# lijrjyan/SDVAR

Measured on AMD Instinct MI355X. Metric: images/s (+ mean accepted tokens/step), VAR-d16 256^2 B=8, d12 draft + d16 verify, per GPU, higher is better.
Workload: dtype f32 (GEMM operands split into 2 fp16 planes to 2^-22, 3 fp16 MFMA products, fp32 accumulate); 1 GPU; BASELINE.json P1: VAR-d16 256^2 B=8/GPU, d12 draft + d16 verify, gamma=2, cfg=1.5 top_k=900 top_p=0.96, acceptance=natural, incl. VQVAE decode (overlapped with the next batch on a 2nd stream); verifier one round behind the draft once gamma = 1; parallelism=1 independent batch shards

## Files before the change

sdvar_amd/csrc/gemm.hip:

```cpp
#include "common.h"
#include "gemm_plan.h"

namespace sdvar {

enum { EPI_BIAS = 0, EPI_BIAS_GELU = 1, EPI_GATED_RES = 2, EPI_PARTIAL = 3 };

constexpr int BK = 32;
constexpr int LDS_STRIDE = BK + 4;

struct GemmArgs {
    const float* X; const float* W; const float* bias; float* out;
    const float* res; const float* gate;
    int M, N, K, ldx, ldo, ldres;
    int rows_per_gate, gate_stride;
    int split, k_per_split;
};

template <int BM, int BN, int WAVES_M, int WAVES_N, int EPI>
__global__ __launch_bounds__(256) void gemm_f32_nt_kernel(GemmArgs a) {
    static_assert(WAVES_M * WAVES_N == 4, "4 waves per workgroup");
    constexpr int WM = BM / WAVES_M, WN = BN / WAVES_N;
    constexpr int TM = WM / 32, TN = WN / 32;
    static_assert(TM >= 1 && TN >= 1, "wave tile too small");
    constexpr int XV = BM / 32, WV = BN / 32;
// ... 59 lines not shown
            for (int i = 0; i < TM; ++i) fa[i] = *reinterpret_cast<const f32x4*>(px + i * 32 * LDS_STRIDE + 8 * c);
#pragma unroll
            for (int j = 0; j < TN; ++j) fb[j] = *reinterpret_cast<const f32x4*>(pw + j * 32 * LDS_STRIDE + 8 * c);
#pragma unroll
            for (int e = 0; e < 4; ++e)
#pragma unroll
                for (int i = 0; i < TM; ++i)
#pragma unroll
                    for (int j = 0; j < TN; ++j)
                        acc[i][j] = __builtin_amdgcn_mfma_f32_32x32x2f32(fa[i][e], fb[j][e], acc[i][j], 0, 0, 0);
        }
        if (kt + 1 < nk) store_tile(buf ^ 1);
        __syncthreads();
    }

#pragma unroll
    for (int j = 0; j < TN; ++j) {
        const int n = n0 + wn * WN + j * 32 + li;
        if (n >= a.N) continue;
        const float bv = (EPI != EPI_PARTIAL && a.bias) ? a.bias[n] : 0.f;
        float* outp = (EPI == EPI_PARTIAL) ? a.out + (size_t)ks * a.M * a.ldo : a.out;
#pragma unroll
        for (int i = 0; i < TM; ++i) {
#pragma unroll
            for (int r = 0; r < 16; ++r) {
                const int m = m0 + wm * WM + i * 32 + (r & 3) + 8 * (r >> 2) + 4 * lh;
                if (m >= a.M) continue;
                float v = acc[i][j][r] + bv;
                if (EPI == EPI_BIAS_GELU) v = gelu_tanh(v);
                if (EPI == EPI_GATED_RES) {
                    const float g = a.gate[(size_t)(m / a.rows_per_gate) * a.gate_stride + n];
                    v = a.res[(size_t)m * a.ldres + n] + v * g;
                }
                outp[(size_t)m * a.ldo + n] = v;
            }
        }
    }
}

template <int EPI>
__global__ __launch_bounds__(256) void splitk_reduce_kernel(const float* __restrict__ ws, int split, const float* __restrict__ bias, float* out,
                                                            const float* res, const float* __restrict__ gate, int M, int N, int ldo, int ldres,
                                                            int rows_per_gate, int gate_stride) {
    const int nv = N >> 2;
    const size_t total = (size_t)M * nv, slab = (size_t)M * N;
    for (size_t i = (size_t)blockIdx.x * blockDim.x + threadIdx.x; i < total; i += (size_t)gridDim.x * blockDim.x) {
        const int m = (int)(i / nv), n = (int)(i % nv) * 4;
        f32x4 acc = *reinterpret_cast<const f32x4*>(ws + (size_t)m * N + n);
        for (int s = 1; s < split; ++s) {
            const f32x4 p = *reinterpret_cast<const f32x4*>(ws + s * slab + (size_t)m * N + n);
            acc[0] += p[0]; acc[1] += p[1]; acc[2] += p[2]; acc[3] += p[3];
        }
#pragma unroll
        for (int e = 0; e < 4; ++e) {
            float v = acc[e] + (bias ? bias[n + e] : 0.f);
            if (EPI == EPI_BIAS_GELU) v = gelu_tanh(v);
            if (EPI == EPI_GATED_RES) v = res[(size_t)m * ldres + n + e] + v * gate[(size_t)(m / rows_per_gate) * gate_stride + n + e];
            out[(size_t)m * ldo + n + e] = v;
        }
    }
}

static thread_local float* g_ws = nullptr;
constexpr size_t WS_FLOATS = (size_t)24 << 20;

static thread_local float* g_ws_model = nullptr;
float* set_splitk_workspace(float* p) { float* old = g_ws_model; g_ws_model = p; return old; }
size_t splitk_workspace_floats() { return WS_FLOATS; }

float* splitk_workspace(size_t* floats) {
    if (floats) *floats = WS_FLOATS;
    if (g_ws_model) return g_ws_model;
    if (!g_ws && hipMalloc((void**)&g_ws, WS_FLOATS * sizeof(float)) != hipSuccess) { set_error("split-K workspace allocation failed"); return nullptr; }
    return g_ws;
}

Variant g_variants[VAR_COUNT] = {
    {"gemm_h4_var", "SDVAR_GEMM_H4_VAR", 3, 0, 3, 3, false, false},
    {"gemm_h2_stages", "SDVAR_GEMM_H2_STAGES", 6, 2, 6, 6, false, false},
    {"gemm_small_pp", "SDVAR_GEMM_SMALL_PP", 2, 0, 2, 2, false, false},
    {"attn_pp_sched", "SDVAR_ATTN_PP_SCHED", 1, 0, 3, 1, false, false},
    {"conv_pp", "SDVAR_CONV_PP", 2, 0, 2, 2, true, false},
    {"conv_tap_reuse", "SDVAR_CONV_TAP_REUSE", 1, 0, 1, 1, true, false},
    {"rowblk", "SDVAR_ROWBLK", 1, 0, 2, 1, false, false},
    {"qkv_fuse", "SDVAR_NO_QKV_FUSE", 1, 0, 1, 1, false, true},
    {"gemm_v2", nullptr, 1, 0, 1, 1, false, false},
    {nullptr, nullptr, 0, 0, 768, 0, false, false},
    {nullptr, nullptr, 0, -64, 64, 0, false, false},
};

template <int BM, int BN, int WAVES_M, int WAVES_N, int EPI>
static int launch_f32_kernel(const GemmArgs& a, int grid, hipStream_t stream) {
    const size_t lds = 2 * (size_t)(BM + BN) * LDS_STRIDE * sizeof(float);
    static LdsOptIn opt_in;
    SDVAR_LDS_OPT_IN(opt_in, lds, (const void*)gemm_f32_nt_kernel<BM, BN, WAVES_M, WAVES_N, EPI>);
    hipLaunchKernelGGL((gemm_f32_nt_kernel<BM, BN, WAVES_M, WAVES_N, EPI>), dim3(grid), dim3(256), lds, stream, a);
    SDVAR_LAUNCH_CHECK();
    return SDVAR_OK;
}

static int launch_reduce(const GemmArgs& a, const float* ws, int split, int epi, hipStream_t stream) {
    return dispatch_epi(epi, [&](auto e) {
        hipLaunchKernelGGL(splitk_reduce_kernel<decltype(e)::value>, dim3(splitk_reduce_grid(a.M, a.N)), dim3(256), 0, stream, ws, split, a.bias, a.out, a.res, a.gate, a.M, a.N, a.ldo, a.ldres,
                           a.rows_per_gate, a.gate_stride);
        SDVAR_LAUNCH_CHECK();
        return SDVAR_OK;
    });
}

template <int BM, int BN, int WAVES_M, int WAVES_N>
static int launch_cfg(const GemmArgs& a, int epi, int split, hipStream_t stream) {
    const int tiles = ((a.M + BM - 1) / BM) * ((a.N + BN - 1) / BN);
    return launch_splitk(a, epi, split, tiles, nullptr,
                         [&](const GemmArgs& x, int grid, auto e) { return launch_f32_kernel<BM, BN, WAVES_M, WAVES_N, decltype(e)::value>(x, grid, stream); },
                         [&](const GemmArgs& x, const float* ws, int sp, int ep) { return launch_reduce(x, ws, sp, ep, stream); });
}

int gemm_f32_nt(const float* X, int ldx, const float* W, const float* bias, float* out, int ldo, int M, int N, int K, int epi,
                const float* res, int ldres, const float* gate, int rows_per_gate, int gate_stride, hipStream_t stream) {
    SDVAR_CHECK_ARG(X && W && out, "gemm: null operand");
    SDVAR_CHECK_ARG(M > 0 && N > 0 && K > 0 && K % BK == 0, "gemm: need K %% 32 == 0 (M=%d N=%d K=%d)", M, N, K);
    SDVAR_CHECK_ARG(ldx >= K && ldx % 4 == 0 && ldo >= N, "gemm: bad leading dims ldx=%d ldo=%d", ldx, ldo);
    SDVAR_CHECK_ARG(((uintptr_t)X % 16) == 0 && ((uintptr_t)W % 16) == 0, "gemm: operands must be 16-byte aligned");
    SDVAR_CHECK_ARG(epi >= EPI_BIAS && epi <= EPI_GATED_RES, "gemm: unknown epilogue %d", epi);
    if (epi == EPI_GATED_RES) SDVAR_CHECK_ARG(res && gate && rows_per_gate > 0 && ldres >= N, "gemm: gated-residual epilogue needs res/gate");
    const GemmArgs a{X, W, bias, out, res, gate, M, N, K, ldx, ldo, ldres, rows_per_gate > 0 ? rows_per_gate : 1, gate_stride, 1, K / BK};
    const GemmPlan p = plan_f32(M, N, K, WS_FLOATS);
    if (p.kernel == 32) return launch_cfg<32, 128, 1, 4>(a, epi, p.split, stream);
    if (p.kernel == 64) return launch_cfg<64, 128, 2, 2>(a, epi, p.split, stream);
    return launch_cfg<128, 128, 2, 2>(a, epi, p.split, stream);
}

}
```

sdvar_amd/csrc/gemm_f16x2.hip:

```cpp
#include <stdio.h>
#include <stdlib.h>

#include "common.h"
#include "gemm_plan.h"

namespace sdvar {

unsigned long long* debug_get_gemm_stamps();

typedef _Float16 f16x8 __attribute__((ext_vector_type(8)));
enum { HEPI_BIAS = 0, HEPI_BIAS_GELU_PLANES = 1, HEPI_GATED_RES = 2, HEPI_PARTIAL = 3, HEPI_QKV = 4 };

#ifdef SDVAR_TIMING_EXPERIMENTS
#define SDVAR_DBG(a, bit) ((a).dbg & (bit))
#else
#define SDVAR_DBG(a, bit) 0
#endif

constexpr int HBK = 32;
constexpr int HBN = 128;

struct QkvEpi {
    const float* scale_mul;
    float* q_out; uint16_t* k_cache; uint16_t* v_cache;
// ... 935 lines not shown
            else asm volatile("s_waitcnt vmcnt(0)" ::: "memory");
        }
        SDVAR_H4_SLOT(7);
        SDVAR_H4_MFMA(2, 0, if (p2) issue_w(t + 2, 2, 3), if (p2) issue_w(t + 2, 3, 4));
        SDVAR_H4_SLOT(8);
    }
    if (wm == 0) __builtin_amdgcn_s_barrier();
#ifdef SDVAR_V4_STAMPS
    wsr[2] = __builtin_amdgcn_s_memrealtime(); wsc[2] = __builtin_amdgcn_s_memtime();
    if (a.stamps && blockIdx.x == 0 && lane == 0 && (wave == 0 || wave == 4)) {
#pragma unroll
        for (int k = 0; k < 9; ++k) a.stamps[16 * (wave >> 2) + k] = stm[k];
    }
#endif
#undef SDVAR_H4_MFMA
#undef SDVAR_H4_SLOT
#undef SDVAR_H4_STAMP

    const float wsi = a.wsi ? *a.wsi : 1.0f;
    if (EPI == HEPI_QKV) {
        const int Cq = a.qk.H * 64, nw = n0 + wn * 64, which = nw / Cq, h = (nw - which * Cq) >> 6;
        if (nw >= a.N) return;
#pragma unroll
        for (int i = 0; i < 4; ++i) {
            const int m = m0 + wm * 128 + i * 32 + li;
            f32x16 v[2];
            float sq = qk_bias_sq(a, acc[i][0], v[0], wsi, nw + 4 * lh);
            sq += qk_bias_sq(a, acc[i][1], v[1], wsi, nw + 32 + 4 * lh);
            if (which != 2) sq += __shfl_xor(sq, 32, 64);
            qk_store_row<2>(a, v, sq, which, h, m, lh, 0);
        }
        return;
    }
    float* outp = (EPI == HEPI_PARTIAL) ? a.out + (size_t)ks * a.M * a.ldo : a.out;
    if (a.vec && n0 + BN <= a.N) {
#pragma unroll
        for (int j = 0; j < 2; ++j)
#pragma unroll
            for (int i = 0; i < 4; ++i) h_store_tile_fast<EPI>(a, outp, acc[i][j], wsi, m0 + wm * 128 + i * 32 + li, n0 + wn * 64 + j * 32 + 4 * lh);
    } else {
#pragma unroll
        for (int j = 0; j < 2; ++j)
#pragma unroll
            for (int i = 0; i < 4; ++i) h_store_tile<EPI>(a, outp, acc[i][j], wsi, m0 + wm * 128 + i * 32 + li, n0 + wn * 64 + j * 32 + 4 * lh);
    }
#ifdef SDVAR_V4_STAMPS
    if (a.stamps && lane == 0 && wave == 0 && (blockIdx.x == 0 || blockIdx.x == gridDim.x - 1)) {
        asm volatile("s_waitcnt vmcnt(0)" ::: "memory");
        wsr[3] = __builtin_amdgcn_s_memrealtime(); wsc[3] = __builtin_amdgcn_s_memtime();
        unsigned long long* o = a.stamps + 32 + (blockIdx.x == 0 ? 0 : 8);
#pragma unroll
        for (int k = 0; k < 4; ++k) { o[k] = wsr[k]; o[4 + k] = wsc[k]; }
    }
#endif
}

typedef float f32x4v __attribute__((ext_vector_type(4)));
#define SDVAR_MFMA3_16(acc, xh, xl, wh, wl)                                            \
    acc = __builtin_amdgcn_mfma_f32_16x16x32_f16(wh, xl, acc, 0, 0, 0);                \
    acc = __builtin_amdgcn_mfma_f32_16x16x32_f16(wl, xh, acc, 0, 0, 0);                \
    acc = __builtin_amdgcn_mfma_f32_16x16x32_f16(wh, xh, acc, 0, 0, 0)

template <int EPI>
__device__ __forceinline__ void h_store4(const GemmHArgs& a, float* outp, const f32x4v& acc, float wsi, int m, int n, bool fast) {
    if (m >= a.M || n >= a.N) return;
    if (!fast) {
#pragma unroll
        for (int e = 0; e < 4; ++e)
            if (n + e < a.N) h_store<EPI>(a, outp, acc[e], wsi, (EPI != HEPI_PARTIAL && a.bias) ? a.bias[n + e] : 0.f, m, n + e);
        return;
    }
    f32x4 v;
    if (EPI != HEPI_PARTIAL && a.bias) {
        const f32x4 bv = *reinterpret_cast<const f32x4*>(a.bias + n);
#pragma unroll
        for (int e = 0; e < 4; ++e) v[e] = __builtin_fmaf(acc[e], wsi, bv[e]);
    } else {
#pragma unroll
        for (int e = 0; e < 4; ++e) v[e] = acc[e] * wsi;
    }
    if (EPI == HEPI_BIAS_GELU_PLANES) {
        float gv[4];
#pragma unroll
        for (int e = 0; e < 4; ++e) gv[e] = gelu_tanh_h(v[e]);
        uint2 wh, wl;
        split4h_pk(gv, wh, wl);
        uint16_t* p0 = a.outp + kb_index(m, n, a.M);
        *reinterpret_cast<uint2*>(p0) = wh; *reinterpret_cast<uint2*>(p0 + a.ops) = wl;
        return;
    }
    if (EPI == HEPI_GATED_RES) {
        const f32x4 rv = *reinterpret_cast<const f32x4*>(a.res + (size_t)m * a.ldres + n);
        const f32x4 gt = *reinterpret_cast<const f32x4*>(a.gate + (size_t)(m / a.rows_per_gate) * a.gate_stride + n);
#pragma unroll
        for (int e = 0; e < 4; ++e) v[e] = rv[e] + v[e] * gt[e];
    }
    *reinterpret_cast<f32x4*>(outp + (size_t)m * a.ldo + n) = v;
}

template <int EPI>
__global__ __launch_bounds__(512, 2) void gemm_f16x2_v5_kernel(GemmHArgs a) {
    extern __shared__ __attribute__((aligned(16))) uint16_t hsm[];
    constexpr int BM = 256, BN = 256;
    const int tiles_m = (a.M + BM - 1) / BM, tiles_n = (a.N + BN - 1) / BN, ntile = tiles_m * tiles_n;
    const int ks = blockIdx.x / ntile;
    const int lid = xcd_remap(blockIdx.x - ks * ntile, ntile);
    const int G = 4, per_group = tiles_m * G;
    const int g = lid / per_group, rem = lid - g * per_group;
    const int gw = min(G, tiles_n - g * G);
    const int tm = rem / gw, tn = g * G + rem % gw;
    const int m0 = tm * BM, n0 = tn * BN;

    const int tid = threadIdx.x, lane = tid & 63, l15 = lane & 15, lq = lane >> 4;
    const int wave = __builtin_amdgcn_readfirstlane(tid >> 6);
    const int wm = wave >> 2, wn = wave & 3;
    const int kt0 = ks * a.k_per_split;
    const int nk = min(a.K / HBK - kt0, a.k_per_split);

    const int dpl = wave >> 2, drow0 = 64 * (wave & 3) + (lane >> 2);
    const int dch = (lane & 3) ^ ((lane >> 4) & 3);
    uint32_t vx[4], vw[4];
#pragma unroll
    for (int e = 0; e < 4; ++e) {
        vx[e] = (uint32_t)(min(m0 + drow0 + 16 * e, a.M - 1) * 32 + 8 * dch) * 2u;
        vw[e] = (uint32_t)(min(n0 + drow0 + 16 * e, a.N - 1) * 32 + 8 * dch) * 2u;
    }
    const char* const bx = reinterpret_cast<const char*>(a.X + (size_t)kt0 * a.M * 32 + (size_t)dpl * a.xps);
    const char* const bw = reinterpret_cast<const char*>(a.W + (size_t)kt0 * a.N * 32 + (size_t)dpl * a.wps);
    const uint32_t lds0 = SDVAR_LDS_ADDR(hsm);
    const uint32_t ldx = lds0 + (uint32_t)(dpl * 16384 + (64 * (wave & 3)) * 64), ldw = ldx + 32768u;
    auto issue_x = [&](int t) {
        const char* src = bx + (size_t)t * a.M * 64;
        const uint32_t dst = ldx + (uint32_t)(t & 1) * 65536u;
#pragma unroll
        for (int e = 0; e < 4; ++e) SDVAR_DMA16(vx[e], src, dst + 1024u * e);
    };
    auto issue_w = [&](int t) {
        const char* src = bw + (size_t)t * a.N * 64;
        const uint32_t dst = ldw + (uint32_t)(t & 1) * 65536u;
#pragma unroll
        for (int e = 0; e < 4; ++e) SDVAR_DMA16(vw[e], src, dst + 1024u * e);
    };

    f32x4v acc[8][4];
#pragma unroll
    for (int i = 0; i < 8; ++i)
#pragma unroll
        for (int j = 0; j < 4; ++j)
#pragma unroll
            for (int r = 0; r < 4; ++r) acc[i][j][r] = 0.f;

    const uint32_t fro = (uint32_t)(l15 * 64 + 16 * (lq ^ ((l15 >> 2) & 3)));
    const uint32_t ax = lds0 + (uint32_t)(wm * 128 * 64) + fro, aw = lds0 + 32768u + (uint32_t)(wn * 64 * 64) + fro;

    issue_w(0); issue_x(0);
    if (nk > 1) { issue_w(1); issue_x(1); asm volatile("s_waitcnt vmcnt(8)" ::: "memory"); }
    else asm volatile("s_waitcnt vmcnt(0)" ::: "memory");
    __builtin_amdgcn_s_barrier();
    if (wm == 1) __builtin_amdgcn_s_barrier();

    f16x8 fx[4][2], fw[4][2];
#define SDVAR_H5_SLOT() do { __builtin_amdgcn_sched_barrier(0); __builtin_amdgcn_s_barrier(); __builtin_amdgcn_sched_barrier(0); } while (0)
#define SDVAR_H5_MFMA(I0, J0)                                                                                              \
    do {                                                                                                                   \
        _Pragma("unroll") for (int i_ = 0; i_ < 4; ++i_)                                                                   \
            _Pragma("unroll") for (int j_ = 0; j_ < 2; ++j_) { SDVAR_MFMA3_16(acc[(I0) + i_][(J0) + j_], fx[i_][0], fx[i_][1], fw[(J0) + j_][0], fw[(J0) + j_][1]); } \
    } while (0)
#pragma unroll 1
    for (int t = 0; t < nk; ++t) {
// ... 890 lines not shown
```

sdvar_amd/csrc/gemm_plan.h:

```cpp
#pragma once
#include <limits.h>
#include <stdlib.h>
#include <string.h>

#include <atomic>
#include <type_traits>

#include "common.h"

namespace sdvar {

enum VariantId { VAR_GEMM_H4, VAR_GEMM_H2_STAGES, VAR_GEMM_SMALL_PP, VAR_ATTN_PP_SCHED, VAR_CONV_PP, VAR_CONV_TAP_REUSE, VAR_ROWBLK, VAR_QKV_FUSE, VAR_GEMM_V2, VAR_FORCE_BM, VAR_FORCE_SPLIT, VAR_COUNT };

struct Variant {
    const char* name;
    const char* env;
    int def, lo, hi, fallback;
    bool env_per_call;
    bool env_switches_off;
    std::atomic<int> set{INT_MIN}, cached{INT_MIN};

    int from_env() const {
        const char* e = env ? getenv(env) : nullptr;
        if (!e) return def;
        if (env_switches_off) return 0;
        const int v = atoi(e);
        return v < lo || v > hi ? fallback : v;
    }
    int get() {
        const int s = set.load(std::memory_order_relaxed);
        if (s != INT_MIN && !env_switches_off) return s;
        int c = env_per_call ? from_env() : cached.load(std::memory_order_relaxed);
        if (c == INT_MIN) { c = from_env(); cached.store(c, std::memory_order_relaxed); }
        return (s == INT_MIN || c == 0) ? c : s;
    }
    void store(int v) { set.store(v, std::memory_order_relaxed); }
    void put(int v) { store(v < 0 ? INT_MIN : v); }
};
extern Variant g_variants[VAR_COUNT];
inline int variant(VariantId id) { return g_variants[id].get(); }
inline int set_variant_by_name(const char* name, int value) {
    for (Variant& v : g_variants) {
        if (!v.name || strcmp(v.name, name)) continue;
        SDVAR_CHECK_ARG(value <= v.hi && (value < 0 || value >= v.lo), "%s %d", name, value);
        v.put(value);
        return SDVAR_OK;
    }
    set_error("debug_set_variant: unknown variant '%s'", name);
    return SDVAR_ERR_ARG;
}

inline bool env_flag(const char* name) { return getenv(name) != nullptr; }
inline bool gemm_no_hybrid() { static const bool v = env_flag("SDVAR_GEMM_NO_HYBRID"); return v; }
inline bool gemm_no_v4() { static const bool v = env_flag("SDVAR_GEMM_NO_V4"); return v; }
inline bool gemm_no_v7() { static const bool v = env_flag("SDVAR_GEMM_NO_V7"); return v; }
inline int gemm_skinny_max() { static const int v = getenv("SDVAR_GEMM_SKINNY_MAX") ? atoi(getenv("SDVAR_GEMM_SKINNY_MAX")) : 80; return v; }
inline bool gemm_trace() { static const bool v = env_flag("SDVAR_GEMM_TRACE"); return v; }

size_t splitk_workspace_floats();
float* splitk_workspace(size_t* floats);

constexpr int PLAN_BK = 32, PLAN_BN = 128;

struct GemmPlan { int kernel; int split; int tail; bool qkv_fused; };

struct QkvEpi;
struct GemmCall { int* defer; const QkvEpi* qkv; int* fused; };

struct GemmCostModel {
    int ntile; int bm[4]; int resident[4];
    double kstep, kfac[4], ppfac[4], lat[5];
    double kover, fix, fixbm, red0, redbw, defbw;
};

constexpr GemmCostModel COST_F32 = {3, {128, 64, 32, 0}, {2, 2, 3, 0}, 64.0 * 16.0, {1.0, 1.03, 1.12, 0.0}, {1.0, 1.0, 1.0, 1.0}, {0.0, 1.35, 1.08, 1.0, 1.0},
                                    0.0, 2500.0, 40.0, 6000.0, 1800.0, 0.0};
constexpr GemmCostModel COST_BF16X3 = {4, {256, 128, 64, 32}, {1, 1, 3, 3}, 384.0, {1.1, 1.0, 1.3, 1.3}, {1.0, 1.0, 1.0, 1.0}, {0.0, 1.2, 1.0, 1.0, 1.0},
                                       260.0, 1500.0, 20.0, 2000.0, 5000.0, 0.0};
constexpr GemmCostModel COST_F16X2 = {4, {256, 128, 64, 32}, {1, 1, 2, 2}, 192.0, {1.0, 1.0, 1.1, 1.8}, {1.0, 1.0, 1.0, 1.0}, {0.0, 1.0, 0.8, 1.0, 1.0},
                                      260.0, 8000.0, 80.0, 4000.0, 5000.0, 2000.0};
constexpr double COST_K4 = 2850.0, COST_FIX4 = 50000.0;

inline GemmPlan plan_tiles(const GemmCostModel& cm, int M, int N, int K, size_t ws_floats, bool allow_hybrid, bool deferred, double* cost = nullptr) {
    const int nkt = K / PLAN_BK, tiles_n = (N + PLAN_BN - 1) / PLAN_BN;
    double best = 1e30;
    GemmPlan p{128, 1, 0, false};
    for (int bi = 0; bi < cm.ntile; ++bi) {
        const int bm = cm.bm[bi], res = cm.resident[bi];
        const int tiles = ((M + bm - 1) / bm) * tiles_n;
        const double ktile = cm.kstep * (bm / 32) * cm.kfac[bi] * cm.ppfac[bi];
        for (int split = 1; split <= 32 && split <= nkt / 2; ++split) {
            if (split > 1 && ((size_t)split * M * N > ws_floats || N % 4)) break;
            const int kps = (nkt + split - 1) / split;
            if ((nkt + kps - 1) / kps != split) continue;
            const long blocks = (long)tiles * split;
// ... 151 lines not shown
```

sdvar_amd/csrc/vae.hip:

```cpp
#include <math.h>

#include <vector>

#include "../../include/sdvar_hip.h"
#include "common.h"

namespace sdvar {

int conv_weight_planes(const float* w, uint16_t* planes, int Cout, int Cin, int taps, size_t plane_stride, int pfmt, const float* scale, hipStream_t stream);
int weight_scale_f16(const float* w, size_t n, float* sc, hipStream_t stream);
int conv_planes(const uint16_t* X, size_t xps, size_t x_rows, int x_row0, const uint16_t* W, size_t wps, int pfmt, const float* wsi, const float* bias, const float* res,
                float* out, int B, int H, int Wd, int N, int Cin, int taps, float* ws, size_t ws_floats, int force_split, double* gn_part, int* gn_done, int up_phase,
                size_t w_phase_stride, hipStream_t stream);
int upconv_weights(const float* w, float* weff, int Cout, int Cin, hipStream_t stream);

__global__ __launch_bounds__(256) void rows_from_nchw_kernel(const float* __restrict__ in, float* __restrict__ out, int B, int C, int H, int W) {
    const size_t total = (size_t)B * H * W * C;
    for (size_t i = (size_t)blockIdx.x * blockDim.x + threadIdx.x; i < total; i += (size_t)gridDim.x * blockDim.x) {
        const int c = (int)(i % C);
        const size_t row = i / C;
        const int x = (int)(row % W), y = (int)((row / W) % H), b = (int)(row / ((size_t)W * H));
        out[i] = in[(((size_t)b * C + c) * H + y) * W + x];
    }
}

__global__ __launch_bounds__(320) void gn_partial_kernel(const float* __restrict__ x, double* __restrict__ part, int C, int H, int W, int rows_per_chunk) {
    __shared__ float sm[2 * 1280];
    const int b = blockIdx.y, chunk = blockIdx.x, nq = C >> 2, npl = 320 / nq;
    const int q = threadIdx.x % nq, pl = threadIdx.x / nq;
    const int y0 = chunk * rows_per_chunk, y1 = min(H, y0 + rows_per_chunk);
    const float* x0 = x + ((size_t)b * H + y0) * W * C;
    const f32x4 K = *reinterpret_cast<const f32x4*>(x0 + 4 * q);
    float s[4] = {0.f, 0.f, 0.f, 0.f}, ss[4] = {0.f, 0.f, 0.f, 0.f};
    const int npix = (y1 - y0) * W;
    for (int p = pl; p < npix; p += npl) {
        const f32x4 v = *reinterpret_cast<const f32x4*>(x0 + (size_t)p * C + 4 * q);
#pragma unroll
        for (int e = 0; e < 4; ++e) { const float d = v[e] - K[e]; s[e] += d; ss[e] += d * d; }
    }
    const int NL = npl * C;
#pragma unroll
    for (int e = 0; e < 4; ++e) { sm[pl * C + 4 * q + e] = s[e]; sm[NL + pl * C + 4 * q + e] = ss[e]; }
    __syncthreads();
    if (threadIdx.x < 32) {
        const int g = threadIdx.x, cpg = C / 32;
        const double n = (double)npix, in = 1.0 / n;
        double a = 0.0, m = 0.0;
        for (int c = g * cpg; c < (g + 1) * cpg; ++c) {
            double s1 = 0.0, s2 = 0.0;
            for (int l = 0; l < npl; ++l) { s1 += (double)sm[l * C + c]; s2 += (double)sm[NL + l * C + c]; }
            const double sc = n * (double)x0[c] + s1;
            a += sc; m += s2 + (sc * sc - s1 * s1) * in;
        }
        double* o = part + (((size_t)b * gridDim.x + chunk) * 32 + g) * 2;
        o[0] = a; o[1] = m - a * a / (n * cpg);
    }
}

__global__ __launch_bounds__(256) void gn_finalize_kernel(const double* __restrict__ part, float* __restrict__ stats, int nchunk, double n_full, double n_last, double eps) {
    __shared__ double sm[2][8][32];
    const int b = blockIdx.x, g = threadIdx.x & 31, sl = threadIdx.x >> 5;
    const double* pb = part + (size_t)b * nchunk * 64 + 2 * g;
    const double if_ = 1.0 / n_full, il = 1.0 / n_last;
    double a = 0.0, m = 0.0;
    for (int c = sl; c < nchunk; c += 8) {
        const double s = pb[(size_t)c * 64];
        a += s; m += pb[(size_t)c * 64 + 1] + s * s * (c == nchunk - 1 ? il : if_);
    }
    sm[0][sl][g] = a; sm[1][sl][g] = m;
    __syncthreads();
    if (sl) return;
    for (int i = 1; i < 8; ++i) { a += sm[0][i][g]; m += sm[1][i][g]; }
    const double count = (nchunk - 1) * n_full + n_last, mean = a / count, var = fmax((m - a * mean) / count, 0.0);
    stats[((size_t)b * 32 + g) * 2] = (float)mean;
    stats[((size_t)b * 32 + g) * 2 + 1] = (float)(1.0 / sqrt(var + eps));
}

static int gn_finalize(const double* part, float* stats, int B, int nchunk, double n_full, double n_last, hipStream_t s) {
    hipLaunchKernelGGL(gn_finalize_kernel, dim3(B), dim3(256), 0, s, part, stats, nchunk, n_full, n_last, 1e-6);
    SDVAR_LAUNCH_CHECK();
    return SDVAR_OK;
}

static int gn_stats_rows(const float* x, double* part, float* stats, int B, int C, int H, int W, hipStream_t s) {
    SDVAR_CHECK_ARG(x && part && stats && B >= 1 && H >= 1 && W >= 1 && C % 32 == 0 && C >= 32 && C <= 1280 && 320 % (C / 4) == 0,
                    "gn_stats: C = %d unsupported ((C/4) must divide 320) or bad shape (B %d H %d W %d)", C, B, H, W);
    const int nch = H < 64 ? H : 64, rpc = (H + nch - 1) / nch, chunks = (H + rpc - 1) / rpc, cpg = C / 32;
    hipLaunchKernelGGL(gn_partial_kernel, dim3(chunks, B), dim3(320), 0, s, x, part, C, H, W, rpc);
    SDVAR_LAUNCH_CHECK();
    return gn_finalize(part, stats, B, chunks, (double)rpc * W * cpg, (double)(H - (chunks - 1) * rpc) * W * cpg, s);
}

static int gn_stats_fused(const double* part, float* stats, int B, int N, int HW, bool up, hipStream_t s) {
    const double n = 256.0 * (N / 32);
    return gn_finalize(part, stats, B, (up ? 4 : 1) * (HW / 256), n, n, s);
}

struct FastDiv { uint32_t mul, sh; };
static FastDiv fastdiv_make(uint32_t d) {
    FastDiv f{0u, 0u};
    uint32_t l = 31;
    while (!((d >> l) & 1u)) --l;
    if ((d & (d - 1)) == 0) { f.mul = 0; f.sh = l - 1; return f; }
    const uint64_t num = (uint64_t)1 << (32 + l);
    uint64_t m = num / d;
    const uint64_t rem = num - m * d;
    m += m;
    const uint64_t twice = rem + rem;
    if (twice >= d || twice < rem) m += 1;
    f.mul = (uint32_t)(m + 1); f.sh = l;
    return f;
}
__device__ __forceinline__ uint32_t fastdiv(uint32_t n, FastDiv f) {
    const uint32_t t = __umulhi(n, f.mul);
    return (((n - t) >> 1) + t) >> f.sh;
}

__global__ __launch_bounds__(256) void prep_planes_kernel(const float* __restrict__ in, const float* __restrict__ stats, const float* __restrict__ gamma,
                                                          const float* __restrict__ beta, uint16_t* __restrict__ outp, size_t ops, int B, int C, int Hi, int Wi,
                                                          int up, int mode, int G, int pfmt, FastDiv dc8, FastDiv dw, FastDiv dh, FastDiv dg) {
    const int Ho = Hi << up, Wo = Wi << up, w2o = Wo + 2, h2o = Ho + 2;
    const uint32_t Mo = (uint32_t)B * h2o * w2o, R = Mo + 2u * (uint32_t)G;
    const uint32_t c8n = (uint32_t)C >> 3, cpg = C / 32;
    const uint32_t total = R * c8n;
    for (uint32_t i = blockIdx.x * blockDim.x + threadIdx.x; i < total; i += gridDim.x * blockDim.x) {
        const uint32_t r = fastdiv(i, dc8), c8 = i - r * c8n;
        float v[8] = {0.f, 0.f, 0.f, 0.f, 0.f, 0.f, 0.f, 0.f};
        bool live = false;
        if (r >= (uint32_t)G && r < (uint32_t)G + Mo) {
            const uint32_t row = r - G;
            const uint32_t ry = fastdiv(row, dw), b = fastdiv(ry, dh);
            const int x = (int)(row - ry * w2o) - 1, y = (int)(ry - b * h2o) - 1;
            if (x >= 0 && x < Wo && y >= 0 && y < Ho) {
                live = true;
                const float* p = in + (((size_t)b * Hi + (y >> up)) * Wi + (x >> up)) * C + 8 * c8;
                const f32x4 a0 = *reinterpret_cast<const f32x4*>(p), a1 = *reinterpret_cast<const f32x4*>(p + 4);
#pragma unroll
                for (int e = 0; e < 4; ++e) { v[e] = a0[e]; v[4 + e] = a1[e]; }
                if (mode & 1) {
                    const f32x4 g0 = *reinterpret_cast<const f32x4*>(gamma + 8 * c8), g1 = *reinterpret_cast<const f32x4*>(gamma + 8 * c8 + 4);
                    const f32x4 b0 = *reinterpret_cast<const f32x4*>(beta + 8 * c8), b1 = *reinterpret_cast<const f32x4*>(beta + 8 * c8 + 4);
                    const float* st = stats + (size_t)b * 64;
#pragma unroll
                    for (int e = 0; e < 8; ++e) {
                        const uint32_t g = cpg == 1 ? 8 * c8 + e : fastdiv(8 * c8 + e, dg);
                        const f32x2p mr = *reinterpret_cast<const f32x2p*>(st + 2 * g);
                        v[e] = ((v[e] - mr[0]) * mr[1]) * (e < 4 ? g0[e & 3] : g1[e & 3]) + (e < 4 ? b0[e & 3] : b1[e & 3]);
                    }
                }
                if (mode & 2) {
#pragma unroll
                    for (int e = 0; e < 8; ++e) v[e] = v[e] * __builtin_amdgcn_rcpf(1.0f + __builtin_amdgcn_exp2f(v[e] * -1.4426950408889634f));
                }
            }
        }
        u32x4 a = {0, 0, 0, 0}, bq = {0, 0, 0, 0}, cq = {0, 0, 0, 0};
        const size_t o = ((size_t)(c8 >> 2) * R + r) * 32 + 8 * (c8 & 3);
        if (pfmt == PLANES_F16X2) {
            if (live) {
                float m = fmaxf(absmax3(v[0], v[1], v[2]), absmax3(v[3], v[4], v[5]));
                m = fmaxf(m, fmaxf(fabsf(v[6]), fabsf(v[7])));
                const bool clampw = __builtin_amdgcn_ballot_w64(m > 65504.0f) != 0ull;
                if (clampw) {
#pragma unroll
                    for (int e = 0; e < 8; ++e) v[e] = clamp_f16_range(v[e]);
                }
#pragma unroll
                for (int e = 0; e < 4; ++e) { uint32_t hw, lw; split2h_pk_raw(v[2 * e], v[2 * e + 1], hw, lw); a[e] = hw; bq[e] = lw; }
            }
            *reinterpret_cast<u32x4*>(outp + o) = a; *reinterpret_cast<u32x4*>(outp + ops + o) = bq;
            continue;
        }
        if (live) split8_packed(v, a, bq, cq);
        *reinterpret_cast<u32x4*>(outp + o) = a; *reinterpret_cast<u32x4*>(outp + ops + o) = bq; *reinterpret_cast<u32x4*>(outp + 2 * ops + o) = cq;
    }
}
static int launch_prep_planes(const float* in, const float* stats, const float* gamma, const float* beta, uint16_t* outp, size_t ops, int B, int C, int Hi, int Wi, int up, int mode,
                              int G, int pfmt, hipStream_t s) {
    const size_t rows = (size_t)B * ((Hi << up) + 2) * ((Wi << up) + 2) + 2 * (size_t)G, total = rows * (C / 8);
    SDVAR_CHECK_ARG(total < ((size_t)1 << 31) && C >= 16 && C % 32 == 0, "vae prep: %zu (row, 8-channel) items exceed the 32-bit index range, or C = %d", total, C);
    const unsigned grid = (unsigned)((total + 255) / 256 < 8192 ? (total + 255) / 256 : 8192);
    hipLaunchKernelGGL(prep_planes_kernel, dim3(grid), dim3(256), 0, s, in, stats, gamma, beta, outp, ops, B, C, Hi, Wi, up, mode, G, pfmt, fastdiv_make((uint32_t)C / 8),
                       fastdiv_make((uint32_t)(Wi << up) + 2), fastdiv_make((uint32_t)(Hi << up) + 2), fastdiv_make(C / 32 >= 2 ? (uint32_t)C / 32 : 2u));
    SDVAR_LAUNCH_CHECK();
    return SDVAR_OK;
}

constexpr int VA_QT = 16, VA_SP = VA_QT + 4;
typedef float f32x2v __attribute__((ext_vector_type(2)));
typedef float f32x4m __attribute__((ext_vector_type(4)));
template <int NKT>
__global__ __launch_bounds__(512) void vae_attn_mfma_kernel(const float* __restrict__ qkv, float* __restrict__ out, int C, int N) {
    extern __shared__ __attribute__((aligned(16))) float vps[];
    const int b = blockIdx.y, q0 = blockIdx.x * 16, tid = threadIdx.x, lane = tid & 63, j = lane & 15, g = lane >> 4;
    const int wave = __builtin_amdgcn_readfirstlane(tid >> 6);
    const int SP = N + 4;
    const float* base = qkv + (size_t)b * N * 3 * C;
    const float scale = 1.0f / sqrtf((float)C);
    {
        f32x4m tot[NKT];
#pragma unroll
        for (int t = 0; t < NKT; ++t) tot[t] = f32x4m{0.f, 0.f, 0.f, 0.f};
        const float* pq = base + (size_t)(q0 + j) * 3 * C + 4 * g;
        const float* pk = base + (size_t)(wave * (N / 8) + j) * 3 * C + C + 4 * g;
        for (int cb = 0; cb < C; cb += 64) {
            f32x4m acc[NKT];
#pragma unroll
            for (int t = 0; t < NKT; ++t) acc[t] = f32x4m{0.f, 0.f, 0.f, 0.f};
#pragma unroll
            for (int sl = 0; sl < 4; ++sl) {
                const int c0 = cb + 16 * sl;
                const f32x4 qv = *reinterpret_cast<const f32x4*>(pq + c0);
                f32x4 kv[NKT];
#pragma unroll
                for (int t = 0; t < NKT; ++t) kv[t] = *reinterpret_cast<const f32x4*>(pk + (size_t)(16 * t) * 3 * C + c0);
#pragma unroll
                for (int t = 0; t < NKT; ++t)
#pragma unroll
                    for (int e = 0; e < 4; ++e) acc[t] = __builtin_amdgcn_mfma_f32_16x16x4f32(qv[e], kv[t][e], acc[t], 0, 0, 0);
            }
#pragma unroll
            for (int t = 0; t < NKT; ++t) tot[t] += acc[t];
        }
#pragma unroll
        for (int t = 0; t < NKT; ++t)
#pragma unroll
            for (int r = 0; r < 4; ++r) vps[(4 * g + r) * SP + wave * (N / 8) + 16 * t + j] = tot[t][r] * scale;
    }
    __syncthreads();
    for (int qi = 2 * wave; qi < 2 * wave + 2; ++qi) {
        float* row = vps + qi * SP;
        float m = -INFINITY;
        for (int k = lane; k < N; k += 64) m = fmaxf(m, row[k]);
        m = wave_max(m);
        float sum = 0.f;
        for (int k = lane; k < N; k += 64) { const float e = expf(row[k] - m); row[k] = e; sum += e; }
        sum = wave_sum(sum);
        const float inv = 1.0f / sum;
        for (int k = lane; k < N; k += 64) row[k] *= inv;
    }
    __syncthreads();
    const float* pp = vps + j * SP + 4 * g;
    for (int grp = wave; grp < C / 64; grp += 8) {
        f32x4m acc[4];
#pragma unroll
        for (int e = 0; e < 4; ++e) acc[e] = f32x4m{0.f, 0.f, 0.f, 0.f};
        const float* pv = base + 2 * C + 64 * grp + 4 * j;
#pragma unroll 4
        for (int k0 = 0; k0 < N; k0 += 16) {
            const f32x4 pr = *reinterpret_cast<const f32x4*>(pp + k0);
            f32x4 vv[4];
#pragma unroll
            for (int mm = 0; mm < 4; ++mm) vv[mm] = *reinterpret_cast<const f32x4*>(pv + (size_t)(k0 + 4 * g + mm) * 3 * C);
#pragma unroll
            for (int mm = 0; mm < 4; ++mm)
#pragma unroll
                for (int e = 0; e < 4; ++e) acc[e] = __builtin_amdgcn_mfma_f32_16x16x4f32(pr[mm], vv[mm][e], acc[e], 0, 0, 0);
        }
#pragma unroll
        for (int r = 0; r < 4; ++r) {
            const int qi = q0 + 4 * g + r;
            *reinterpret_cast<f32x4*>(out + ((size_t)b * N + qi) * C + 64 * grp + 4 * j) = f32x4{acc[0][r], acc[1][r], acc[2][r], acc[3][r]};
        }
    }
}

// ... 902 lines not shown
```

Measured before the change: 187.7 images/s.

## Add row-grouped VAE plane-prep kernel with per-wave channel slots and cached group stats

Adds a new prep_planes_rows_kernel, enabled by default through a new variant, that gives each wave a fixed channel slot and strides over 16-row groups. Each lane keeps gamma/beta in registers and reloads the group-norm mean/rstd only when the batch index changes. Stores from a wave now cover contiguous rows of the plane layout, replacing the per-item index decomposition and the scattered stores of the original kernel. The old kernel also gains debug-only knobs behind SDVAR_TIMING_EXPERIMENTS, and the GEMM GELU epilogue gets similar probe switches. The new path requires C >= 32 and caps the grid at 1280 workgroups, which may limit parallelism on large tensors.

```diff
diff --git a/sdvar_amd/csrc/gemm.hip b/sdvar_amd/csrc/gemm.hip
--- a/sdvar_amd/csrc/gemm.hip
+++ b/sdvar_amd/csrc/gemm.hip
@@ -165,6 +165,7 @@
     {"attn_pp_sched", "SDVAR_ATTN_PP_SCHED", 1, 0, 3, 1, false, false},
     {"conv_pp", "SDVAR_CONV_PP", 2, 0, 2, 2, true, false},
     {"conv_tap_reuse", "SDVAR_CONV_TAP_REUSE", 1, 0, 1, 1, true, false},
+    {"plane_row_stores", "SDVAR_PLANE_ROW_STORES", 1, 0, 1, 1, true, false},
     {"rowblk", "SDVAR_ROWBLK", 1, 0, 2, 1, false, false},
     {"qkv_fuse", "SDVAR_NO_QKV_FUSE", 1, 0, 1, 1, false, true},
     {"gemm_v2", nullptr, 1, 0, 1, 1, false, false},
diff --git a/sdvar_amd/csrc/gemm_f16x2.hip b/sdvar_amd/csrc/gemm_f16x2.hip
--- a/sdvar_amd/csrc/gemm_f16x2.hip
+++ b/sdvar_amd/csrc/gemm_f16x2.hip
@@ -1041,9 +1041,11 @@
     if (EPI == HEPI_BIAS_GELU_PLANES) {
         float gv[4];
 #pragma unroll
-        for (int e = 0; e < 4; ++e) gv[e] = gelu_tanh_h(v[e]);
+        for (int e = 0; e < 4; ++e) gv[e] = SDVAR_DBG(a, 16) ? v[e] : gelu_tanh_h(v[e]);
         uint2 wh, wl;
-        split4h_pk(gv, wh, wl);
+        if (SDVAR_DBG(a, 16)) { wh = uint2{__float_as_uint(gv[0]), __float_as_uint(gv[1])}; wl = uint2{__float_as_uint(gv[2]), __float_as_uint(gv[3])}; }
+        else split4h_pk(gv, wh, wl);
+        if (SDVAR_DBG(a, 32) && (wh.x ^ wh.y ^ wl.x ^ wl.y) != 0x12345679u) return;
         uint16_t* p0 = a.outp + kb_index(m, n, a.M);
         *reinterpret_cast<uint2*>(p0) = wh; *reinterpret_cast<uint2*>(p0 + a.ops) = wl;
         return;
diff --git a/sdvar_amd/csrc/gemm_plan.h b/sdvar_amd/csrc/gemm_plan.h
--- a/sdvar_amd/csrc/gemm_plan.h
+++ b/sdvar_amd/csrc/gemm_plan.h
@@ -10,7 +10,7 @@
 
 namespace sdvar {
 
-enum VariantId { VAR_GEMM_H4, VAR_GEMM_H2_STAGES, VAR_GEMM_SMALL_PP, VAR_ATTN_PP_SCHED, VAR_CONV_PP, VAR_CONV_TAP_REUSE, VAR_ROWBLK, VAR_QKV_FUSE, VAR_GEMM_V2, VAR_FORCE_BM, VAR_FORCE_SPLIT, VAR_COUNT };
+enum VariantId { VAR_GEMM_H4, VAR_GEMM_H2_STAGES, VAR_GEMM_SMALL_PP, VAR_ATTN_PP_SCHED, VAR_CONV_PP, VAR_CONV_TAP_REUSE, VAR_PLANE_ROW_STORES, VAR_ROWBLK, VAR_QKV_FUSE, VAR_GEMM_V2, VAR_FORCE_BM, VAR_FORCE_SPLIT, VAR_COUNT };
 
 struct Variant {
     const char* name;
diff --git a/sdvar_amd/csrc/vae.hip b/sdvar_amd/csrc/vae.hip
--- a/sdvar_amd/csrc/vae.hip
+++ b/sdvar_amd/csrc/vae.hip
@@ -4,6 +4,7 @@
 
 #include "../../include/sdvar_hip.h"
 #include "common.h"
+#include "gemm_plan.h"
 
 namespace sdvar {
 
@@ -116,9 +117,14 @@
     return (((n - t) >> 1) + t) >> f.sh;
 }
 
+#ifdef SDVAR_TIMING_EXPERIMENTS
+#define SDVAR_PDBG(dbg, bit) ((dbg) & (bit))
+#else
+#define SDVAR_PDBG(dbg, bit) 0
+#endif
 __global__ __launch_bounds__(256) void prep_planes_kernel(const float* __restrict__ in, const float* __restrict__ stats, const float* __restrict__ gamma,
                                                           const float* __restrict__ beta, uint16_t* __restrict__ outp, size_t ops, int B, int C, int Hi, int Wi,
-                                                          int up, int mode, int G, int pfmt, FastDiv dc8, FastDiv dw, FastDiv dh, FastDiv dg) {
+                                                          int up, int mode, int G, int pfmt, FastDiv dc8, FastDiv dw, FastDiv dh, FastDiv dg, int dbg) {
     const int Ho = Hi << up, Wo = Wi << up, w2o = Wo + 2, h2o = Ho + 2;
     const uint32_t Mo = (uint32_t)B * h2o * w2o, R = Mo + 2u * (uint32_t)G;
     const uint32_t c8n = (uint32_t)C >> 3, cpg = C / 32;
@@ -134,17 +140,21 @@
             if (x >= 0 && x < Wo && y >= 0 && y < Ho) {
                 live = true;
                 const float* p = in + (((size_t)b * Hi + (y >> up)) * Wi + (x >> up)) * C + 8 * c8;
-                const f32x4 a0 = *reinterpret_cast<const f32x4*>(p), a1 = *reinterpret_cast<const f32x4*>(p + 4);
+                f32x4 a0, a1;
+                if (SDVAR_PDBG(dbg, 4)) { a0 = f32x4{(float)i, 1.f, (float)c8, 3.f} * 1e-6f; a1 = a0 + 1.f; }
+                else { a0 = *reinterpret_cast<const f32x4*>(p); a1 = *reinterpret_cast<const f32x4*>(p + 4); }
 #pragma unroll
                 for (int e = 0; e < 4; ++e) { v[e] = a0[e]; v[4 + e] = a1[e]; }
                 if (mode & 1) {
-                    const f32x4 g0 = *reinterpret_cast<const f32x4*>(gamma + 8 * c8), g1 = *reinterpret_cast<const f32x4*>(gamma + 8 * c8 + 4);
-                    const f32x4 b0 = *reinterpret_cast<const f32x4*>(beta + 8 * c8), b1 = *reinterpret_cast<const f32x4*>(beta + 8 * c8 + 4);
+                    const bool nop = SDVAR_PDBG(dbg, 8) != 0;
+                    const f32x4 one = {1.f, 1.f, 1.f, 1.f};
+                    const f32x4 g0 = nop ? one : *reinterpret_cast<const f32x4*>(gamma + 8 * c8), g1 = nop ? one : *reinterpret_cast<const f32x4*>(gamma + 8 * c8 + 4);
+                    const f32x4 b0 = nop ? one : *reinterpret_cast<const f32x4*>(beta + 8 * c8), b1 = nop ? one : *reinterpret_cast<const f32x4*>(beta + 8 * c8 + 4);
                     const float* st = stats + (size_t)b * 64;
 #pragma unroll
                     for (int e = 0; e < 8; ++e) {
                         const uint32_t g = cpg == 1 ? 8 * c8 + e : fastdiv(8 * c8 + e, dg);
-                        const f32x2p mr = *reinterpret_cast<const f32x2p*>(st + 2 * g);
+                        const f32x2p mr = nop ? f32x2p{0.5f, 1.5f} : *reinterpret_cast<const f32x2p*>(st + 2 * g);
                         v[e] = ((v[e] - mr[0]) * mr[1]) * (e < 4 ? g0[e & 3] : g1[e & 3]) + (e < 4 ? b0[e & 3] : b1[e & 3]);
                     }
                 }
@@ -152,6 +162,87 @@
 #pragma unroll
                     for (int e = 0; e < 8; ++e) v[e] = v[e] * __builtin_amdgcn_rcpf(1.0f + __builtin_amdgcn_exp2f(v[e] * -1.4426950408889634f));
                 }
+            }
+        }
+        u32x4 a = {0, 0, 0, 0}, bq = {0, 0, 0, 0}, cq = {0, 0, 0, 0};
+        const size_t o = SDVAR_PDBG(dbg, 1) ? (size_t)i * 8 : ((size_t)(c8 >> 2) * R + r) * 32 + 8 * (c8 & 3);
+        if (pfmt == PLANES_F16X2) {
+            if (live) {
+                float m = fmaxf(absmax3(v[0], v[1], v[2]), absmax3(v[3], v[4], v[5]));
+                m = fmaxf(m, fmaxf(fabsf(v[6]), fabsf(v[7])));
+                const bool clampw = __builtin_amdgcn_ballot_w64(m > 65504.0f) != 0ull;
+                if (clampw) {
+#pragma unroll
+                    for (int e = 0; e < 8; ++e) v[e] = clamp_f16_range(v[e]);
+                }
+#pragma unroll
+                for (int e = 0; e < 4; ++e) { uint32_t hw, lw; split2h_pk_raw(v[2 * e], v[2 * e + 1], hw, lw); a[e] = hw; bq[e] = lw; }
+            }
+            if (SDVAR_PDBG(dbg, 2) && (a[0] ^ a[1] ^ a[2] ^ a[3] ^ bq[0] ^ bq[1] ^ bq[2] ^ bq[3]) != 0x12345679u) continue;
+            *reinterpret_cast<u32x4*>(outp + o) = a; *reinterpret_cast<u32x4*>(outp + ops + o) = bq;
+            continue;
+        }
+        if (live) split8_packed(v, a, bq, cq);
+        *reinterpret_cast<u32x4*>(outp + o) = a; *reinterpret_cast<u32x4*>(outp + ops + o) = bq; *reinterpret_cast<u32x4*>(outp + 2 * ops + o) = cq;
+    }
+}
+
+__global__ __launch_bounds__(256) void prep_planes_rows_kernel(const float* __restrict__ in, const float* __restrict__ stats, const float* __restrict__ gamma,
+                                                               const float* __restrict__ beta, uint16_t* __restrict__ outp, size_t ops, int B, int C, int Hi, int Wi,
+                                                               int up, int mode, int G, int pfmt, FastDiv dw, FastDiv dh, FastDiv dg, uint32_t rg_stride) {
+    const int Ho = Hi << up, Wo = Wi << up, w2o = Wo + 2, h2o = Ho + 2;
+    const uint32_t Mo = (uint32_t)B * h2o * w2o, R = Mo + 2u * (uint32_t)G, ngrp = (R + 15u) >> 4;
+    const uint32_t cpg = C / 32;
+    const uint32_t lane = threadIdx.x & 63u, gw = blockIdx.x * 4u + (threadIdx.x >> 6);
+    const uint32_t slot = gw / cpg, c8 = 4u * (gw - slot * cpg) + (lane & 3u);
+    f32x2p gm[4], bt[4], mean[4], rstd[4];
+    uint32_t bcur = 0xFFFFFFFFu;
+#pragma unroll
+    for (int e = 0; e < 4; ++e) { gm[e] = f32x2p{1.f, 1.f}; bt[e] = mean[e] = f32x2p{0.f, 0.f}; rstd[e] = f32x2p{1.f, 1.f}; }
+    if (mode & 1) {
+        const f32x4 g0 = *reinterpret_cast<const f32x4*>(gamma + 8 * c8), g1 = *reinterpret_cast<const f32x4*>(gamma + 8 * c8 + 4);
+        const f32x4 b0 = *reinterpret_cast<const f32x4*>(beta + 8 * c8), b1 = *reinterpret_cast<const f32x4*>(beta + 8 * c8 + 4);
+        gm[0] = f32x2p{g0[0], g0[1]}; gm[1] = f32x2p{g0[2], g0[3]}; gm[2] = f32x2p{g1[0], g1[1]}; gm[3] = f32x2p{g1[2], g1[3]};
+        bt[0] = f32x2p{b0[0], b0[1]}; bt[1] = f32x2p{b0[2], b0[3]}; bt[2] = f32x2p{b1[0], b1[1]}; bt[3] = f32x2p{b1[2], b1[3]};
+    }
+    for (uint32_t rg = slot; rg < ngrp; rg += rg_stride) {
+        const uint32_t r = 16u * rg + (lane >> 2);
+        if (r >= R) continue;
+        float v[8] = {0.f, 0.f, 0.f, 0.f, 0.f, 0.f, 0.f, 0.f};
+        bool live = false;
+        if (r >= (uint32_t)G && r < (uint32_t)G + Mo) {
+            const uint32_t row = r - G;
+            const uint32_t ry = fastdiv(row, dw), b = fastdiv(ry, dh);
+            const int x = (int)(row - ry * w2o) - 1, y = (int)(ry - b * h2o) - 1;
+            if (x >= 0 && x < Wo && y >= 0 && y < Ho) {
+                live = true;
+                const float* p = in + (((size_t)b * Hi + (y >> up)) * Wi + (x >> up)) * C + 8 * c8;
+                const f32x4 a0 = *reinterpret_cast<const f32x4*>(p), a1 = *reinterpret_cast<const f32x4*>(p + 4);
+                f32x2p vv[4] = {f32x2p{a0[0], a0[1]}, f32x2p{a0[2], a0[3]}, f32x2p{a1[0], a1[1]}, f32x2p{a1[2], a1[3]}};
+                if (mode & 1) {
+                    if (b != bcur) {
+                        const float* st = stats + (size_t)b * 64;
+#pragma unroll
+                        for (int e = 0; e < 4; ++e) {
+                            const uint32_t ga = cpg == 1 ? 8 * c8 + 2 * e : fastdiv(8 * c8 + 2 * e, dg), gb = cpg == 1 ? 8 * c8 + 2 * e + 1 : fastdiv(8 * c8 + 2 * e + 1, dg);
+                            const f32x2p m0 = *reinterpret_cast<const f32x2p*>(st + 2 * ga), m1 = *reinterpret_cast<const f32x2p*>(st + 2 * gb);
+                            mean[e] = f32x2p{m0[0], m1[0]}; rstd[e] = f32x2p{m0[1], m1[1]};
+                        }
+                        bcur = b;
+                    }
+#pragma unroll
+                    for (int e = 0; e < 4; ++e) vv[e] = ((vv[e] - mean[e]) * rstd[e]) * gm[e] + bt[e];
+                }
+                if (mode & 2) {
+#pragma unroll
+                    for (int e = 0; e < 4; ++e) {
+                        const f32x2p t = vv[e] * -1.4426950408889634f;
+                        const f32x2p d = 1.0f + f32x2p{__builtin_amdgcn_exp2f(t[0]), __builtin_amdgcn_exp2f(t[1])};
+                        vv[e] = vv[e] * f32x2p{__builtin_amdgcn_rcpf(d[0]), __builtin_amdgcn_rcpf(d[1])};
+                    }
+                }
+#pragma unroll
+                for (int e = 0; e < 4; ++e) { v[2 * e] = vv[e][0]; v[2 * e + 1] = vv[e][1]; }
             }
         }
         u32x4 a = {0, 0, 0, 0}, bq = {0, 0, 0, 0}, cq = {0, 0, 0, 0};
@@ -175,13 +266,27 @@
         *reinterpret_cast<u32x4*>(outp + o) = a; *reinterpret_cast<u32x4*>(outp + ops + o) = bq; *reinterpret_cast<u32x4*>(outp + 2 * ops + o) = cq;
     }
 }
+
 static int launch_prep_planes(const float* in, const float* stats, const float* gamma, const float* beta, uint16_t* outp, size_t ops, int B, int C, int Hi, int Wi, int up, int mode,
                               int G, int pfmt, hipStream_t s) {
-    const size_t rows = (size_t)B * ((Hi << up) + 2) * ((Wi << up) + 2) + 2 * (size_t)G, total = rows * (C / 8);
-    SDVAR_CHECK_ARG(total < ((size_t)1 << 31) && C >= 16 && C % 32 == 0, "vae prep: %zu (row, 8-channel) items exceed the 32-bit index range, or C = %d", total, C);
+    const size_t rows = (size_t)B * ((Hi << up) + 2) * ((Wi << up) + 2) + 2 * (size_t)G, total = (rows + 15) / 16 * 16 * (C / 8);
+    SDVAR_CHECK_ARG(total < ((size_t)1 << 31) && C >= 32 && C % 32 == 0, "vae prep: %zu (row, 8-channel) items exceed the 32-bit index range, or C = %d", total, C);
+    const FastDiv dw = fastdiv_make((uint32_t)(Wi << up) + 2), dh = fastdiv_make((uint32_t)(Hi << up) + 2), dg = fastdiv_make(C / 32 >= 2 ? (uint32_t)C / 32 : 2u);
+    if (variant(VAR_PLANE_ROW_STORES) == 1) {
+        const unsigned cpg = (unsigned)C / 32, waves = (unsigned)((rows + 15) / 16) * cpg, cap = 1280 / cpg * cpg;
+        unsigned grid = ((waves + 3) / 4 + cpg - 1) / cpg * cpg;
+        if (grid > cap) grid = cap;
+        hipLaunchKernelGGL(prep_planes_rows_kernel, dim3(grid), dim3(256), 0, s, in, stats, gamma, beta, outp, ops, B, C, Hi, Wi, up, mode, G, pfmt, dw, dh, dg, 4 * grid / cpg);
+        SDVAR_LAUNCH_CHECK();
+        return SDVAR_OK;
+    }
     const unsigned grid = (unsigned)((total + 255) / 256 < 8192 ? (total + 255) / 256 : 8192);
-    hipLaunchKernelGGL(prep_planes_kernel, dim3(grid), dim3(256), 0, s, in, stats, gamma, beta, outp, ops, B, C, Hi, Wi, up, mode, G, pfmt, fastdiv_make((uint32_t)C / 8),
-                       fastdiv_make((uint32_t)(Wi << up) + 2), fastdiv_make((uint32_t)(Hi << up) + 2), fastdiv_make(C / 32 >= 2 ? (uint32_t)C / 32 : 2u));
+#ifdef SDVAR_TIMING_EXPERIMENTS
+    static const int dbg = getenv("SDVAR_PREP_DBG") ? atoi(getenv("SDVAR_PREP_DBG")) : 0;
+#else
+    const int dbg = 0;
+#endif
+    hipLaunchKernelGGL(prep_planes_kernel, dim3(grid), dim3(256), 0, s, in, stats, gamma, beta, outp, ops, B, C, Hi, Wi, up, mode, G, pfmt, fastdiv_make((uint32_t)C / 8), dw, dh, dg, dbg);
     SDVAR_LAUNCH_CHECK();
     return SDVAR_OK;
 }
```

Measured after the change: 188.1 images/s (median of 3 runs). No clear change (+0.2%).
